# LorenzoNajt/FlipComplexityEmpirical

Measured on AMD Instinct MI355X. Metric: flip proposals/sec (node) 40x40 grid k=2, 1/2/4/8 MI355X; % LDS/HBM roofline, higher is better.
Workload: dtype int8

## Files before the change

flipcomplexityempirical_amd/csrc/fc_capi.cpp:

```cpp
#include <algorithm>
#include <cstdio>
#include <cstdlib>
#include <cstring>
#include <memory>
#include <new>
#include <string>
#include <vector>

#include "fc_run.h"

struct fc_graph {
    fc::HostGraph h;
};

namespace {

constexpr int kWaveSlots = 64;
thread_local std::string g_err;
thread_local char g_seed_kname[96] = {0};

}

int fc::fail(int code, const std::string &msg) {
    g_err = msg;
// ... 305 lines not shown
    if (!r) return fail(FC_ERR_ARG, "fc_run_set_tape: null run");
    if (r->d_sbits && tape && n_draws > 0)
        return fail(FC_ERR_ARG, "fc_run_set_tape: replay tapes need the node stream (FC_STREAM_NODE)");
    HIP_TRY(hipSetDevice(r->p.device));
    r->d_tape.release();
    r->tape_draws = 0;
    if (!tape || n_draws <= 0) return FC_OK;
    if (int rc = r->d_tape.upload(tape, (size_t)r->n_chains * (size_t)n_draws * 6)) return rc;
    r->tape_draws = n_draws;
    return FC_OK;
}

int fc_run_set_initial_wait(fc_run *r, const uint32_t *words) {
    if (!r || !words) return fail(FC_ERR_ARG, "fc_run_set_initial_wait: null argument");
    if (!(r->p.diag_mask & FC_DIAG_WAIT)) return fail(FC_ERR_ARG, "fc_run_set_initial_wait: FC_DIAG_WAIT is off");
    if (r->p.proposal == FC_PROPOSE_RECOM) return fail(FC_ERR_UNSUPPORTED, "fc_run_set_initial_wait: flip runs only");
    std::vector<fc::ChainScalars> sc;
    if (int rc = download_scalars(r, 0, r->n_chains, sc)) return rc;
    for (const auto &s : sc)
        if (s.steps != 0 || s.draw != 0) return fail(FC_ERR_ARG, "fc_run_set_initial_wait: a chain has stepped");
    for (int32_t c = 0; c < r->n_chains; ++c) {
        fc::ChainScalars &s = sc[c];
        const int64_t w = fc::geom_from(fc::u53(words[2 * c], words[2 * c + 1]), r->log1mp[s.nb]);
        s.sum_wait += w - s.wait_cur;
        s.wait_cur = w;
    }
    HIP_TRY(hipMemcpy(r->d_sc, sc.data(), sc.size() * sizeof(sc[0]), hipMemcpyHostToDevice));
    return FC_OK;
}

#ifdef FC_PHASE_PROF
static int dump_prof(fc_run *r, hipStream_t s) {
    if (const char *path = std::getenv("FC_PROF_OUT")) {
        std::vector<int64_t> h((size_t)r->n_chains * fc::kProfSlots);
        HIP_TRY(hipStreamSynchronize(s));
        HIP_TRY(hipMemcpy(h.data(), r->d_prof, h.size() * 8, hipMemcpyDeviceToHost));
        if (FILE *f = std::fopen(path, "ab")) {
            std::fwrite(h.data(), 8, h.size(), f);
            std::fclose(f);
        }
    }
    return FC_OK;
}
#endif

static fc::KParams flip_params(const fc_run *r, int64_t n_steps, int64_t max_draws) {
    fc::KParams k{};
    k.graph = r->d_graph;
    k.ring_eid = r->d_ring_eid;
    k.n = r->g.n;
    k.n_edges = r->g.n_edges;
    k.n_chains = r->n_chains;
    k.k = r->p.k;
    k.popk = r->d_popk;
    k.all_exact = r->g.n_exact == r->g.n ? 1 : 0;
    k.dgraph = r->dgraph ? 1 : 0;
    k.mcnt = r->d_mcnt;
    k.ngk = r->d_ngk;
    k.wmax = r->wmax > 0 ? r->wmax : 1;
    k.wdyn = r->p.k > 2 && r->wmax <= 0 ? 1 : 0;
    k.nfh = r->d_nfh;
    k.band = r->d_sbits ? 1 : 0;
    k.sbits = r->d_sbits;
    k.band_step0 = 1;
    while (k.band_step0 * 2 < r->words) k.band_step0 *= 2;
    k.chain_lds_bytes = r->chain_lds_bytes;
    k.words = r->words;
    k.lab_words = fc::bfs_lab_words(r->g.n);
    k.lemire_thresh = (uint32_t)((1ull << 32) % (uint64_t)r->g.n);
    k.chain_id_offset = r->p.chain_id_offset;
    k.seed_lo = (uint32_t)r->p.seed;
    k.seed_hi = (uint32_t)(r->p.seed >> 32);
    k.pop_lo = (int32_t)r->p.pop_lo;
    k.pop_hi = (int32_t)r->p.pop_hi;
    k.n_steps = n_steps;
    k.max_draws = max_draws > 0 ? max_draws : 65536 * std::max<int64_t>(n_steps, 1);
    k.assign = r->d_assign;
    k.fcnt = r->d_fcnt;
    k.sc = r->d_sc;
    k.thresh = r->d_thresh;
    k.log1mp = r->d_log1mp;
    k.labels = r->d_labels;
    k.diag = r->p.diag_mask;
    k.flags = r->p.flags;
    k.cut_hist = r->d_cut_hist;
    k.nb_hist = r->d_nb_hist;
    k.nb_w = r->nb_w;
    k.nb_pairs = (r->p.flags & FC_FLAG_NB_PAIRS) && r->p.k > 2;
    k.edge_acc = r->d_edge_acc;
    k.num_flips = r->d_num_flips;
    k.part_sum = r->d_part_sum;
    k.last_flipped = r->d_last_flipped;
    k.flip_count = r->d_flip_count;
    k.occ_acc = r->d_occ_acc;
    k.last_accept = r->d_last_accept;
    k.trace = r->d_trace;
    k.trace_chains = r->p.trace_chains;
    k.trace_cap = r->p.trace_cap;
    k.tape = r->d_tape;
    k.tape_draws = r->tape_draws;
    k.events = r->d_events;
    k.ev_cap = r->ev_cap;
    k.hit_lo = r->p.hit_lo;
    k.hit_hi = r->p.hit_hi;
    k.nsub = r->tune.nsub;
    k.hit_stop = r->tune.hit_stop;
    k.par_min = r->tune.par_min;
    k.multi_flip = r->tune.multi ? r->mf_marks : 0;
    k.wait_q = r->tune.wait_q;
    k.wpb = r->tune.wpb;
    k.coop = r->tune.coop ? 1 : 0;
    k.variant = r->variant ? 1 : 0;
    k.accept = r->p.accept;
    k.con_valid = r->p.con_valid;
    k.con_accept = r->p.con_accept;
    if (r->variant) k.par_min = kWaveSlots + 1;
    for (int i = 0; i < 3; ++i) {
        k.prio_nb[i] = r->tune.prio_div[0] > 0 && r->p.k == 2 ? k.n / r->tune.prio_div[i] : 0;
        k.prio_th[i] = r->tune.prio_th[i];
    }
    return k;
}

static fc::RecomParams recom_params(const fc_run *r, int64_t n_steps, int64_t max_draws, int64_t *prof) {
    fc::RecomParams q{};
    q.graph = r->d_graph;
    q.nbe = r->d_nbe;
    q.eslot = r->d_eslot;
    q.nb_d = r->nb_d;
    q.eu = r->d_eu;
    q.ev = r->d_ev;
    q.n = r->g.n;
    q.n_edges = r->g.n_edges;
    q.n_chains = r->n_chains;
    q.chain_lds_bytes = r->chain_lds_bytes;
    q.chain_id_offset = r->p.chain_id_offset;
    q.seed_lo = (uint32_t)r->p.seed;
    q.seed_hi = (uint32_t)(r->p.seed >> 32);
    q.pop_lo = (int32_t)r->p.pop_lo;
    q.pop_hi = (int32_t)r->p.pop_hi;
    q.pop_target = r->p.recom_pop_target;
    q.epsilon = r->p.recom_epsilon;
    q.node_repeats = r->p.recom_node_repeats > 0 ? r->p.recom_node_repeats : 1;
    q.max_attempts = r->p.recom_max_attempts > 0 ? r->p.recom_max_attempts : 10000;
    q.n_steps = n_steps;
    q.max_draws = max_draws > 0 ? max_draws : 1024 * std::max<int64_t>(n_steps, 1);
    q.assign = r->d_assign;
    q.sc = r->d_sc;
    q.accept_thresh = r->d_recom_thresh;
    q.trace = (fc_recom_record *)r->d_trace.get();
    q.trace_chains = r->p.trace_chains;
    q.trace_cap = r->p.trace_cap;
    q.prof = prof;
    return q;
}

static int take_event_slot(fc_run *r, size_t *slot) {
    if (r->n_launch_events < r->launch_events.size()) {
        *slot = (r->ev_head + r->n_launch_events) % r->launch_events.size();
        ++r->n_launch_events;
    } else if (r->launch_events.size() < fc::kMaxLaunchEvents) {
        hipEvent_t a, b;
        HIP_TRY(hipEventCreate(&a));
        HIP_TRY(hipEventCreate(&b));
        r->launch_events.emplace_back(a, b);
        *slot = r->launch_events.size() - 1;
        ++r->n_launch_events;
// ... 180 lines not shown
```

flipcomplexityempirical_amd/csrc/fc_device.h:

```cpp
#pragma once
#include <hip/hip_runtime.h>
#include <stdint.h>

#include "fc_internal.h"
#include "fc_philox.h"
#include "fc_ring.h"

namespace fc {
namespace dev {

__device__ __forceinline__ void compiler_fence() { asm volatile("" ::: "memory"); }
__device__ __forceinline__ void wave_sync() { asm volatile("s_waitcnt lgkmcnt(0)" ::: "memory"); }

#ifdef FC_PHASE_PROF
#ifdef FC_PHASE_SYNC
#define FC_STAMP(t)                                                    \
    asm volatile("s_waitcnt vmcnt(0) lgkmcnt(0)" ::: "memory");        \
    const int64_t t = (int64_t)__builtin_amdgcn_s_memtime()
#else
#define FC_STAMP(t) const int64_t t = (int64_t)__builtin_amdgcn_s_memtime()
#endif
#define FC_PROF(i, x) \
    do { if (lane == 0) atomicAdd((unsigned long long *)&prof_acc[i], (unsigned long long)(int64_t)(x)); } while (0)
#else
// ... 7 lines not shown
__device__ __forceinline__ int rl32(int x, int lane) { return __builtin_amdgcn_readlane(x, lane); }
__device__ __forceinline__ uint32_t rlu(uint32_t x, int lane) { return (uint32_t)__builtin_amdgcn_readlane((int)x, lane); }

__device__ __forceinline__ int64_t rl64(int64_t x, int lane) {
    const uint32_t lo = rlu((uint32_t)x, lane), hi = rlu((uint32_t)((uint64_t)x >> 32), lane);
    return (int64_t)(((uint64_t)hi << 32) | lo);
}
template <typename... T>
__device__ __forceinline__ void wave_sum64_all(T &...x) {
#pragma unroll
    for (int off = 32; off >= 1; off >>= 1) ((x += __shfl_xor((long long)x, off)), ...);
}
__device__ __forceinline__ int64_t wave_sum64(int64_t x) {
    wave_sum64_all(x);
    return x;
}

template <int CTRL>
__device__ __forceinline__ int32_t dpp_pair(int32_t x) {
    return __builtin_amdgcn_update_dpp(x, x, CTRL, 0xf, 0xf, false);
}
constexpr int kQuadSwap1 = 0xB1;
constexpr int kQuadSwap2 = 0x4E;
constexpr int kRowHalfMirror = 0x141;
constexpr int kRowMirror = 0x140;

__device__ __forceinline__ int32_t row0_sum(int32_t x) {
    x += dpp_pair<kQuadSwap1>(x);
    x += dpp_pair<kQuadSwap2>(x);
    x += dpp_pair<kRowHalfMirror>(x);
    x += dpp_pair<kRowMirror>(x);
    return rl32(x, 0);
}
__device__ __forceinline__ int32_t min_lanes32(int32_t x) {
    x = min(x, dpp_pair<kQuadSwap1>(x));
    x = min(x, dpp_pair<kQuadSwap2>(x));
    x = min(x, dpp_pair<kRowHalfMirror>(x));
    x = min(x, dpp_pair<kRowMirror>(x));
    return min(rl32(x, 0), rl32(x, 16));
}

__device__ __forceinline__ int count_below(uint64_t m) {
    return (int)__builtin_amdgcn_mbcnt_hi((uint32_t)(m >> 32), __builtin_amdgcn_mbcnt_lo((uint32_t)m, 0u));
}

template <int CTRL>
__device__ __forceinline__ int dpp_mov(int x) {
    return __builtin_amdgcn_update_dpp(0, x, CTRL, 0xf, 0xf, false);
}

__device__ __forceinline__ int wave_scan_incl(int x) {
    x += dpp_mov<0x111>(x);
    x += dpp_mov<0x112>(x);
    x += dpp_mov<0x114>(x);
    x += dpp_mov<0x118>(x);
    x += __builtin_amdgcn_update_dpp(0, x, 0x142, 0xa, 0xf, false);
    x += __builtin_amdgcn_update_dpp(0, x, 0x143, 0xc, 0xf, false);
    return x;
}

__device__ __forceinline__ int select_bit64(uint64_t x, int r) {
    uint32_t y = (uint32_t)x;
    int pos = 0, c = __popc(y);
    if (r >= c) { r -= c; y = (uint32_t)(x >> 32); pos = 32; }
    c = __popc(y & 0xffffu);
    if (r >= c) { r -= c; y >>= 16; pos += 16; }
    c = __popc(y & 0xffu);
    if (r >= c) { r -= c; y >>= 8; pos += 8; }
    c = __popc(y & 0xfu);
    if (r >= c) { r -= c; y >>= 4; pos += 4; }
    c = __popc(y & 0x3u);
    if (r >= c) { r -= c; y >>= 2; pos += 2; }
    return pos + (r >= (int)(y & 1u) ? 1 : 0);
}

__device__ __forceinline__ int kth_set_bit(uint64_t x, int k) {
    for (int i = 1; i < k; ++i) x &= x - 1;
    return __builtin_ctzll(x);
}

template <int RMAX>
__device__ __forceinline__ int ring_entry(const uint32_t (&ring)[RMAX / 2], int i) {
    return (int)((ring[i >> 1] >> (16 * (i & 1))) & 0xffffu);
}

using fc::one_run;
using fc::one_run_flat;

__device__ __forceinline__ int deal_chain(const KParams &p, int lane) {
    int cc = 0;
    if (lane == 0) {
        uint32_t hw, xcc;
        asm volatile("s_getreg_b32 %0, hwreg(HW_REG_HW_ID)" : "=s"(hw));
        asm volatile("s_getreg_b32 %0, hwreg(HW_REG_XCC_ID)" : "=s"(xcc));
        const uint32_t key = ((xcc & 7u) << 12) | ((hw >> 4) & 0xfffu);
        const uint32_t slot = atomicAdd(&p.deal[key], 1u);
        const uint32_t C = (uint32_t)p.n_chains;
        for (uint32_t k = 0; k < 4; ++k) {
            const uint32_t q = (slot + k) & 3u;
            const uint32_t lo = q * C / 4u, hi = (q + 1u) * C / 4u;
            const uint32_t i = atomicAdd(&p.deal[kDealKeys + q], 1u);
            if (lo + i < hi) {
                cc = (int)p.order[lo + i];
                break;
            }
        }
    }
    return __builtin_amdgcn_readfirstlane(__shfl(cc, 0));
}

constexpr int kBfsList = 512;
struct BfsScratch {
    uint32_t *lab;
    uint32_t *mm;
    uint32_t *cm;
    int32_t *lcnt;
    uint16_t *list;
    uint64_t *vis;
    uint64_t *front;
    uint64_t *nxt;
    int lab_words;
    int W;
    int64_t *prof;
};

__device__ __forceinline__ uint32_t or_reduce(uint32_t x) {
#pragma unroll
    for (int off = 32; off >= 1; off >>= 1) x |= (uint32_t)__shfl_xor((int)x, off);
    return x;
}

template <int RMAX>
__device__ __forceinline__ bool wave_bfs(const NodeRec<RMAX> *__restrict__ G, const int8_t *a, const BfsScratch &S,
                                         int lane, int vf, int A, int my_target, int64_t &levels) {
    const int W = S.W;
    uint8_t *const lab = (uint8_t *)S.lab;
    for (int i = lane; i < W; i += kWave) {
        S.vis[i] = 0;
        S.front[i] = 0;
        S.nxt[i] = 0;
    }
    if (lane < 16) {
        S.mm[lane] = 0;
        S.cm[lane] = 1u << lane;
    }
    const bool src = my_target >= 0;
    const uint64_t SM = __ballot(src);
    const int ns = __popcll(SM);
    wave_sync();
    if (ns <= 1) return true;
    if (src) {
        const uint32_t lab_me = (uint32_t)count_below(SM);
        lab[my_target] = (uint8_t)lab_me;
        atomicOr((unsigned long long *)&S.vis[my_target >> 6], 1ull << (my_target & 63));
        S.list[lab_me] = (uint16_t)my_target;
    }
    if (lane == 0) atomicOr((unsigned long long *)&S.vis[vf >> 6], 1ull << (vf & 63));
    const uint32_t all = (uint32_t)((1ull << ns) - 1ull);
    uint32_t comp = lane < 16 ? (1u << lane) : 0u;
    bool spill_in = false;
    int fcur = ns;
    wave_sync();
    for (int cur = 0;; cur ^= 1) {
        ++levels;
        uint32_t live = 0;
        bool merged = false, spill_out = false;
// ... 387 lines not shown
```

flipcomplexityempirical_amd/csrc/fc_flip2.hip:

```cpp
#include <hip/hip_runtime.h>

#include <cstdio>
#include <cstdlib>
#include <algorithm>

#include "fc_device.h"
#include "fc_internal.h"
#include "fc_philox.h"
#include "fc_tally.h"

namespace fc {

using namespace dev;

#ifndef FC_PRIO_EVERY_LOG2
#define FC_PRIO_EVERY_LOG2 4
#endif
static_assert(sizeof(KParams) % 8 == 0, "flip2_kernel's second argument sits at sizeof(KParams)");
template <bool FULL>
__device__ __forceinline__ PhiloxKeys batch_keys(PhiloxKeys keys) {
    typedef const unsigned char __attribute__((address_space(4))) *KernArg;
    if constexpr (FULL) {
        KernArg ka = (KernArg)__builtin_amdgcn_kernarg_segment_ptr();
        asm volatile("" : "+s"(ka));
        return *(const PhiloxKeys __attribute__((address_space(4))) *)(ka + sizeof(KParams));
    } else {
        asm volatile("" : "+s"(keys));
        return keys;
    }
}

template <int RMAX, int NSUB, bool FULL, bool SEARCH, bool XTRA, bool BAND>
__global__ __launch_bounds__(256, (RMAX == 8 ? 4 : 1)) void flip2_kernel(KParams p, PhiloxKeys keys) {
    static_assert(FULL || !XTRA, "XTRA is a FULL instance");
    constexpr int kRV = BAND ? NSUB : 4;
    extern __shared__ __attribute__((aligned(16))) unsigned char smem[];
    const int lane = (int)(threadIdx.x & 63u);
    const int wv = __builtin_amdgcn_readfirstlane((int)(threadIdx.x >> 6));
    const int wave = (int)blockIdx.x * (int)(blockDim.x >> 6) + wv;
    if (wave >= p.n_chains) return;
    const int c = p.order ? deal_chain(p, lane) : wave;

    const int n = p.n;
    const int npad = (n + 15) & ~15;
    unsigned char *base = smem + (size_t)wv * p.chain_lds_bytes;
    int8_t *a = (int8_t *)base;
    uint8_t *fcnt = base + npad;
    uint64_t *T = (uint64_t *)(base + 2 * npad);
    BfsScratch bs{};
    bs.vis = (uint64_t *)(T + (2 * RMAX + 2));
    bs.front = bs.vis + p.words;
    bs.nxt = bs.front + p.words;
    bs.W = p.words;
    bs.prof = nullptr;
    uint32_t *slot = (uint32_t *)(bs.nxt + p.words);
    uint8_t *smark = (uint8_t *)(slot + 5 * 64);
    uint8_t *nmark = smark + npad;
    uint8_t *const dum = nmark + npad + (lane & 15);
#define FC_ST(cond, ref, val) (*((cond) ? (uint8_t *)&(ref) : dum) = (uint8_t)(val))
    uint64_t *q_d = (uint64_t *)(nmark + npad + 16);
    uint32_t *q_nb = (uint32_t *)(q_d + kWaitQ), *q_run = q_nb + kWaitQ;
    uint32_t *q_v = q_run + kWaitQ, *q_c = q_v + kWaitQ;
    uint64_t *misc = (uint64_t *)(q_c + kWaitQ);
    uint64_t *const sb = misc + 5;
    const NodeRec<RMAX> *__restrict__ G = (const NodeRec<RMAX> *)p.graph;

    {
        const uint4 *ga = (const uint4 *)(p.assign + (size_t)c * npad);
        const uint4 *gf = (const uint4 *)(p.fcnt + (size_t)c * npad);
        for (int i = lane; i < npad / 16; i += kWave) {
            ((uint4 *)a)[i] = ga[i];
            ((uint4 *)fcnt)[i] = gf[i];
        }
        if (lane < 2 * RMAX + 1) T[lane] = p.thresh[(size_t)c * (2 * RMAX + 1) + lane];
        for (int i = lane; i < npad / 4 + 2; i += kWave) ((uint64_t *)smark)[i] = ~0ull;
        if (BAND && lane < p.words) sb[lane] = p.sbits[(size_t)c * p.words + lane];
    }
    ChainScalars *scp = p.sc + c;
    uint64_t draw = scp->draw;
    const int64_t steps_in = scp->steps;
    int64_t trace_len = FULL ? scp->trace_len : 0;
    int64_t ev_len = FULL ? scp->ev_len : 0, hit_time = FULL ? scp->hit_time : 0;
    int cut = scp->cut, nb = scp->nb;
    int pops0 = scp->pops[0], pops1 = scp->pops[1];
    const int pop_lo = scp->pop_lo, pop_hi = scp->pop_hi;
    int ng0 = scp->ngamma[0], ng1 = scp->ngamma[1];
    int64_t wait_cur = scp->wait_cur;
    int qn = 0;
    int last_flip = scp->last_flip;
    int stuck = 0;
    int rem = (int)p.n_steps;
    uint64_t draw_cap = draw + (uint64_t)p.max_draws;
    if (XTRA && p.tape && draw_cap > (uint64_t)p.tape_draws) draw_cap = (uint64_t)p.tape_draws;
    const uint32_t chain_gid = p.chain_id_offset + (uint32_t)c;
    const bool force_bfs = (p.flags & FC_FLAG_FORCE_BFS) != 0;
    const bool want_wait = (p.diag & FC_DIAG_WAIT) != 0;
    const bool trace_on = XTRA && p.trace && c < p.trace_chains;
    const bool defer = (!FULL && !BAND) || ((want_wait || FULL) && !trace_on && !(XTRA && p.tape));

    int64_t acc_cut = 0, acc_nb = 0, acc_wait = 0, acc_cut2 = 0, acc_nb2 = 0;
    int n_acc = 0, n_ic = 0, n_ip = 0;
    int64_t cnt64 = 0;
    auto cnt_fold = [&]() {
        cnt64 += lane == 0 ? n_acc : lane == 1 ? n_ic : lane == 2 ? n_ip : 0;
        n_acc = n_ic = n_ip = 0;
    };
#ifdef FC_PHASE_PROF
    int64_t *prof_acc = (int64_t *)(base + p.chain_lds_bytes - kProfSlots * 8);
    if (lane < kProfSlots) prof_acc[lane] = 0;
#endif
    wave_sync();
    uint32_t nS = 1u, thrS = 0u;
    auto band_count = [&]() {
        const int cw = lane < p.words ? (int)__popcll(sb[lane]) : 0;
        nS = (uint32_t)rl32(wave_scan_incl(cw), kWave - 1);
        thrS = (0u - nS) % nS;
// ... 398 lines not shown
        while (pos < end) {
            FC_PROF(6, 1);
            FC_STAMP(t_it0);
#ifdef FC_PHASE_PROF
            if (first_it) FC_PROF(27, t_it0 - t_c);
            first_it = false;
#endif
            asm volatile("" : "+v"(st), "+v"(inA), "+v"(tmask), "+v"(nbr), "+v"(delta), "+v"(nA), "+v"(av), "+v"(pv),
                         "+v"(v), "+v"(off_l));
            const bool hit = (st & LF_HIT) != 0, acc = (st & LF_ACC) != 0, s_lin = (st & LF_SLIN) != 0,
                       s_cyc = (st & LF_SCYC) != 0, exact = SEARCH ? (st & LF_EXACT) != 0 : true,
                       gam = (st & LF_GAM) != 0, has = (st & LF_HAS) != 0;
            const bool prop = hit & (lane >= pos) & (lane < end);
            const bool bd = SEARCH && (st & ST_BD) != 0, br = SEARCH && (st & ST_BR) != 0, nz = nA != 0;
            const bool okT = bd ? br : (nz & s_lin);
            const bool okN = bd ? br : (nz & ((exact & gam) ? s_cyc : s_lin));
            const bool known = bd | !nz | exact | s_lin;
            const bool ok = ((av ? ng0 : ng1) > 0) ? okT : okN;
            const int pa = av ? pops1 : pops0, pb = av ? pops0 : pops1;
            const bool popok = (pa - pv >= pop_lo) & (pb + pv <= pop_hi);
            bool valid = prop & known & ok & popok;
            bool acc_now = acc;
            bool inv_contig = !ok;
            if constexpr (XTRA) {
                if (p.variant) {
                    const int gm = gam ? 1 : 0;
                    const bool b_ok = ((av ? ng1 : ng0) - gm > 0) && ((av ? ng0 : ng1) + gm > 0);
                    const bool f_ok = !(st & LF_FRZ);
                    auto pass = [&](uint32_t M) {
                        return (!(M & FC_CON_CONTIG) || ok) && (!(M & FC_CON_POP) || popok) &&
                               (!(M & FC_CON_BOUNDARY) || b_ok) && (!(M & FC_CON_FIXED) || f_ok);
                    };
                    valid = prop && known && pass(p.con_valid);
                    inv_contig = (p.con_valid & FC_CON_CONTIG) && !ok;
                    bool au = acc;
                    if (p.accept == FC_ACCEPT_UNIFORM) {
                        au = true;
                    } else if (p.accept == FC_ACCEPT_ANNEAL) {
                        int dnb_l = nA == 0 ? -1 : 0;
#pragma unroll
                        for (int i = 0; i < RMAX; ++i) {
                            const int oc = fcnt[cell[i]];
                            const bool nb_i = (nbr >> i) & 1u;
                            dnb_l += nb_i ? (int)(((inA >> i) & 1u) && oc == 0) - (int)(((tmask >> i) & 1u) && oc == 1) : 0;
                        }
                        const double bw = __longlong_as_double((long long)T[delta + RMAX]);
                        const double bound = bw * ((double)(nb + dnb_l) / (double)nb);
                        au = (double)mant53(w1, w2) * 0x1p-53 < bound;
                    }
                    acc_now = pass(p.con_accept) && au;
                }
            }
            const uint64_t C0 = __ballot(valid && acc_now);
            FC_STAMP(t_it1);
            FC_PROF(8, t_it1 - t_it0);
            if (__popcll(C0) >= p.par_min) {
                FC_PROF(12, 1);
                const bool cand0 = valid && acc;
                const int dp_l = dp_of(), dg_l = dg_of();
                const int x0 = cand0 ? dp_l : 0;
                const int P = wave_scan_incl(x0) - x0;
                const int Gp = count_below(__ballot(cand0 && dg_l > 0)) - count_below(__ballot(cand0 && dg_l < 0));
                const bool ok1 = ((av ? ng0 + Gp : ng1 - Gp) > 0) ? okT : okN;
                const int q0 = pops0 + P, q1 = pops1 - P;
                const bool valid1 = prop & known & ok1 & ((av ? q1 : q0) - pv >= pop_lo) &
                                    ((av ? q0 : q1) + pv <= pop_hi);
                const bool cand1 = valid1 && acc;
                const uint64_t MM = __ballot(prop && cand1 != cand0);
                const uint64_t UU = __ballot(prop && !known);
                int sg = end;
                if (MM) sg = min(sg, __builtin_ctzll(MM) + 1);
                const int u = UU ? __builtin_ctzll(UU) : kWave;
                if (u < sg) sg = u;
                uint64_t VAL = __ballot(valid1) & lane_range(pos, sg);
                bool last_step = false;
                if (__popcll(VAL) >= rem) {
                    sg = kth_set_bit(VAL, rem) + 1;
                    VAL &= bits_below(sg);
                    last_step = true;
                }
                const uint64_t K = __ballot(cand1) & lane_range(pos, sg);
                int x = kWave;
                bool stale_seg = false;
                if (K) {
                    const bool inK = (K >> lane) & 1ull;
                    st |= inK ? LF_WROTE : 0u;
                    bool need = inK;
                    int ms = 0xff, mk[kRV];
                    uint32_t gtm = 0xffffu, ltm = 0u;
                    for (;;) {
                        FC_PROF(21, 1);
                        FC_ST(need && ms > lane, smark[v], lane);
                        const uint32_t wm = need ? (nbr & gtm) : 0u;
#pragma unroll
                        for (int i = 0; i < RMAX; ++i) FC_ST((wm >> i) & 1u, nmark[cell[i]], lane);
                        compiler_fence();
                        ms = smark[v];
                        int mn[RMAX];
#pragma unroll
                        for (int i = 0; i < RMAX; ++i) mn[i] = nmark[cell[i]];
#pragma unroll
                        for (int r = 0; r < kRV; ++r) mk[r] = nmark[rv[r] < 0 ? 0 : (rv[r] & 0xffff)];
                        gtm = 0u;
                        ltm = 0u;
#pragma unroll
                        for (int i = 0; i < RMAX; ++i) {
                            gtm |= (uint32_t)(mn[i] > lane) << i;
                            ltm |= (uint32_t)(mn[i] < lane) << i;
                        }
                        const bool again = (ms > lane) | ((nbr & gtm) != 0u);
                        need = need & again;
                        if (!__any(need)) break;
                    }
                    FC_STAMP(t_mk);
                    FC_PROF(18, t_mk - t_it1);
                    bool conf = (ms < lane) | (inK & ((nbr & ltm) != 0u));
#pragma unroll
                    for (int i = 0; i < RMAX; ++i) conf |= (int)smark[cell[i]] < lane;
                    conf &= has;
                    const uint64_t XX = __ballot(conf && lane > pos && lane < end);
                    if (XX) {
                        x = __builtin_ctzll(XX);
                        stale_seg = true;
                        FC_PROF(13, 1);
                    }
                    int t = trunc_off;
#pragma unroll
                    for (int r = 0; r < kRV; ++r) {
                        const bool tr = (rv[r] >= 0) & (mk[r] < x) & (mk[r] < (rv[r] >> 16));
                        const uint64_t TR = __ballot(tr);
                        if (TR) t = min(t, rv_off(r, __builtin_ctzll(TR)));
                    }
                    if (t < trunc_off) {
                        trunc_off = t;
                        const int e2 = __popcll(__ballot(has && off_l < t));
                        if (e2 < x) x = e2;
                        if (e2 < end) end = e2;
                        FC_PROF(14, 1);
                    }
                }
                FC_STAMP(t_cf);
                FC_PROF(19, t_cf - t_it1);
                int ce = min(sg, x);
                bool seg_out = false;
                if constexpr (BAND) {
                    const uint64_t K0 = K & bits_below(ce);
                    if (K0) {
                        bool out = false;
                        if ((K0 >> lane) & 1ull) {
#pragma unroll
                            for (int i = 0; i < RMAX; ++i) {
                                const int u = cell[i];
                                const uint32_t oc = fcnt[u];
                                const uint64_t swd = sb[u >> 6];
                                out |= ((nbr & inA) >> i & 1u) && oc == 0u && !((swd >> (u & 63)) & 1ull);
                            }
                        }
                        const uint64_t IV = __ballot(out);
                        if (IV) {
                            ce = __builtin_ctzll(IV) + 1;
                            seg_out = true;
                            if (ce < sg) last_step = false;
                        }
                    }
                }
                if (x < sg) last_step = false;
                if (prop && lane < ce) st |= valid1 ? (cand1 ? (ST_VS | ST_AC) : ST_VS) : (ok1 ? ST_IP : ST_IC);
                rem -= __popcll(VAL & bits_below(ce));
                const uint64_t AP = K & bits_below(ce);
                if (AP) {
                    FC_PROF(7, __popcll(AP));
                    const bool me = (AP >> lane) & 1ull;
                    int oldc[RMAX];
#pragma unroll
                    for (int i = 0; i < RMAX; ++i) oldc[i] = fcnt[cell[i]];
                    compiler_fence();
                    int dnb = 0;
                    const uint32_t nbm = me ? nbr : 0u;
#pragma unroll
                    for (int i = 0; i < RMAX; ++i) {
                        const int nw = oldc[i] + 2 * (int)((inA >> i) & 1u) - 1;
                        const uint32_t nb_i = (nbm >> i) & 1u;
                        FC_ST(nb_i, fcnt[cell[i]], nw);
                        dnb += (min(nw, 1) - min(oldc[i], 1)) & -(int)nb_i;
                    }
                    FC_ST(me, *(uint8_t *)&a[v], 1 - av);
                    FC_ST(me, fcnt[v], nA);
                    const int pkd = me ? ((delta + 32) | ((dnb + 32) << 16)) : 0;
                    const int S = wave_scan_incl(pkd);
                    const int cntA = count_below(AP) + 1;
                    cut_after = me ? cut + (S & 0xffff) - 32 * cntA : cut_after;
                    nb_after = me ? nb + (S >> 16) - 32 * cntA : nb_after;
                    const int L = 63 - __builtin_clzll(AP);
                    cut = rl32(cut_after, L);
                    nb = rl32(nb_after, L);
                    const int dP = rl32(P + dp_l, L), dG = rl32(Gp + dg_l, L);
                    pops0 += dP;
                    pops1 -= dP;
                    ng0 += dG;
                    ng1 -= dG;
                    last_flip = rl32(v, L);
                    compiler_fence();
                }
                if (st & LF_WROTE) {
                    smark[v] = 0xff;
#pragma unroll
                    for (int i = 0; i < RMAX; ++i) nmark[cell[i]] = 0xff;
                    st &= ~LF_WROTE;
                }
                FC_STAMP(t_sg1);
                FC_PROF(11, t_sg1 - t_it1);
                pos = ce;
                if (BAND && seg_out) rebuild = true;
                if (last_step) {
                    end = pos;
                    target_hit = true;
                    break;
                }
                if (BAND && seg_out) {
                    end = pos;
                    trunc_off = rl32(off_l, pos - 1) + 1;
                    break;
                }
                if (pos >= end) break;
                if (stale_seg && AP) {
                    reeval(pos, -1, 0u);
                    FC_STAMP(t_sg2);
                    FC_PROF(29, t_sg2 - t_sg1);
                    continue;
                }
                if (SEARCH && u == pos) {
                    const bool res = run_bfs(u);
                    if (lane == u) st |= ST_BD | (res ? ST_BR : 0u);
                }
                FC_STAMP(t_sg3);
                FC_PROF(29, t_sg3 - t_sg1);
                continue;
            }
            const uint64_t VAL = __ballot(valid);
            const uint64_t EV = C0 | __ballot(prop && !known);
            const int f = EV ? __builtin_ctzll(EV) : end;
            const uint64_t segv = VAL & bits_below(f);
            const int nvalid = __popcll(segv);
            const uint32_t bits = valid ? ST_VS : (inv_contig ? ST_IC : ST_IP);
            if (nvalid >= rem) {
                const int e = kth_set_bit(segv, rem);
                st |= (prop & (lane <= e)) ? bits : 0u;
                rem = 0;
                end = e + 1;
                target_hit = true;
                break;
            }
            st |= (prop & (lane < f)) ? bits : 0u;
            rem -= nvalid;
            pos = f;
            if (f >= end) {
                FC_STAMP(t_fx);
                FC_PROF(25, t_fx - t_it1);
                break;
            }
            if (SEARCH && !((VAL >> f) & 1ull)) {
                const bool res = run_bfs(f);
                if (lane == f) st |= ST_BD | (res ? ST_BR : 0u);
                continue;
            }
            FC_PROF(7, 1);
            FC_STAMP(t_ap0);
            FC_PROF(9, t_ap0 - t_it1);
            const int vf = rl32(v, f), Af = rl32(av, f), pvf = rl32(pv, f), df = rl32(delta, f);
            const uint32_t inAf = rlu(inA, f), nbrf = rlu(nbr, f), tmf = rlu(tmask, f);
            const bool gamf = rl32((int)gam, f) != 0;
            uint32_t rw[RMAX / 2];
#pragma unroll
            for (int k2 = 0; k2 < RMAX / 2; ++k2) rw[k2] = rlu(rec.ring[k2], f);
            uint32_t sel = rw[0];
#pragma unroll
            for (int k2 = 1; k2 < RMAX / 2; ++k2) sel = ((lane >> 1) == k2) ? rw[k2] : sel;
            const int my_e = (int)((sel >> (16 * (lane & 1))) & 0xffffu);
            const bool is_nbr = lane < RMAX && ((nbrf >> lane) & 1u);
            const int dlt = (int)((inAf >> lane) & 1u) - (int)((tmf >> lane) & 1u);
            const int old = fcnt[my_e];
            FC_ST(is_nbr, fcnt[my_e], old + dlt);
            const bool enter = is_nbr & (dlt > 0) & (old == 0);
            const bool leave = is_nbr & (dlt < 0) & (old == 1);
            bool outS = false;
            if constexpr (BAND) {
                const uint64_t swd = sb[my_e >> 6];
                outS = enter && !((swd >> (my_e & 63)) & 1ull);
            }
            if (lane == 0) {
// ... 220 lines not shown
                }
                trace_len += __popcll(PM);
            }
        }
        if (!defer && ACCM) wait_cur = rl64(my_wait, 63 - __builtin_clzll(ACCM));
        int consumed;
        if (target_hit) {
            consumed = rl32(off_l, end - 1) + 1;
        } else {
            consumed = end < ns ? rl32(off_l, end) : gen;
            if (trunc_off < consumed) consumed = trunc_off;
        }
        draw += (uint64_t)consumed;
        if constexpr (BAND) {
            if (rebuild) {
                FC_STAMP(t_rb0);
                band_rebuild();
                FC_STAMP(t_rb1);
                FC_PROF(22, 1);
                FC_PROF(23, t_rb1 - t_rb0);
            }
        }
        FC_PROF(24, ns);
        compiler_fence();
        FC_STAMP(t_e);
        FC_PROF(4, t_e - t_d);
    }
    if (defer && qn > 0) wait_flush();
    FC_STAMP(t_loop1);
    FC_PROF(0, t_loop1 - t_loop0);
    if (p.ctime && lane == 0) p.ctime[c] = (uint32_t)min(draw - scp->draw, (uint64_t)0xffffffffu);
    if (p.eta && rem == 0 && lane == 0) {
        const uint64_t el = __builtin_amdgcn_s_memrealtime() - misc[0];
        atomicMax(&p.eta[p.eta_parity], (uint32_t)min(el * 1024ull / (uint64_t)max((int)p.n_steps, 1), 0xffffffffull));
    }
#ifdef FC_PHASE_PROF
    wave_sync();
    if (p.prof && lane == 0)
        for (int i = 0; i < kProfSlots; ++i) p.prof[(size_t)c * kProfSlots + i] = prof_acc[i];
#endif

    {
        uint4 *ga = (uint4 *)(p.assign + (size_t)c * npad);
        uint4 *gf = (uint4 *)(p.fcnt + (size_t)c * npad);
        for (int i = lane; i < npad / 16; i += kWave) {
            ga[i] = ((const uint4 *)a)[i];
            gf[i] = ((const uint4 *)fcnt)[i];
        }
        if (BAND && lane < p.words) p.sbits[(size_t)c * p.words + lane] = sb[lane];
    }
    cnt_fold();
    const int taken = (int)p.n_steps - rem;
    const int64_t cnt_acc = rl64(cnt64, 0), cnt_ic = rl64(cnt64, 1), cnt_ip = rl64(cnt64, 2);
    const int64_t cnt_prop = (int64_t)taken + cnt_ic + cnt_ip;
    wave_sum64_all(acc_cut, acc_nb, acc_wait, acc_cut2, acc_nb2);
    if (FULL && p.tl_len && lane == 0) p.tl_len[c] = (int64_t)misc[3];
    if (lane == 0) {
        scp->draw = draw;
        scp->steps = steps_in + taken;
        scp->proposals += cnt_prop;
        scp->accepted += cnt_acc;
        scp->inv_contig += cnt_ic;
        scp->inv_pop += cnt_ip;
        if (FULL) {
            scp->trace_len = trace_len;
            scp->ev_len = ev_len;
            scp->hit_time = hit_time;
        }
        scp->sum_cut += acc_cut;
        scp->sum_nb += acc_nb;
        scp->sum_wait += acc_wait;
        scp->sum_cut2 += acc_cut2;
        scp->sum_nb2 += acc_nb2;
        scp->cut = cut;
        scp->nb = nb;
        scp->pops[0] = pops0;
        scp->pops[1] = pops1;
        scp->ngamma[0] = ng0;
        scp->ngamma[1] = ng1;
        scp->wait_cur = wait_cur;
        scp->last_flip = last_flip;
        scp->stuck = stuck;
    }
}

int launch_flip2(const KParams &p, const uint32_t *pkeys, int ring_max, void *stream, char *name, size_t name_cap) {
    const int wpb = p.wpb;
    const int blocks = (p.n_chains + wpb - 1) / wpb;
    const size_t lds = (size_t)p.chain_lds_bytes * wpb;
    hipStream_t s = (hipStream_t)stream;
    const dim3 grid(blocks), block(kWave * wpb);
    const PhiloxKeys keys = (PhiloxKeys)(uintptr_t)pkeys;
    const bool full = p.tape || p.trace || (p.diag & ~(uint32_t)FC_DIAG_WAIT) || p.hit_lo <= p.hit_hi || p.variant;
    const bool xtra = p.tape || p.trace || p.variant;
    const bool search = !p.all_exact || (p.flags & FC_FLAG_FORCE_BFS);
#define FC_LAUNCH2B(R, S, F, X, Y, B)                                                                      \
    do {                                                                                                    \
        if (name)                                                                                           \
            snprintf(name, name_cap, "fc::flip2_kernel<%d, %d, %s, %s, %s, %s>", R, S, F ? "true" : "false", \
                     X ? "true" : "false", Y ? "true" : "false", B ? "true" : "false");                    \
        launch_lds(flip2_kernel<R, S, F, X, Y, B>, grid, block, lds, s, p, keys);                           \
    } while (0)
#define FC_LAUNCH2(R, S, F, X, Y)                        \
    do {                                                 \
        if (p.band) FC_LAUNCH2B(R, S, F, X, Y, true);    \
        else FC_LAUNCH2B(R, S, F, X, Y, false);          \
    } while (0)
#define FC_SEARCH2(R, S, F, Y)                    \
    do {                                          \
        if (search) FC_LAUNCH2(R, S, F, true, Y);  \
        else FC_LAUNCH2(R, S, F, false, Y);        \
    } while (0)
#define FC_FULL2(R, S)                                \
    do {                                              \
        if (xtra) FC_SEARCH2(R, S, true, true);        \
        else if (full) FC_SEARCH2(R, S, true, false);  \
        else FC_SEARCH2(R, S, false, false);           \
    } while (0)
#define FC_NSUB2(R)                                \
    switch (p.nsub) {                              \
        case 1: FC_FULL2(R, 1); break;             \
        case 2: FC_FULL2(R, 2); break;             \
        case 4: FC_FULL2(R, 4); break;             \
        default: return (int)hipErrorInvalidValue; \
    }
    if (ring_max == 8) {
        FC_NSUB2(8)
    } else if (ring_max == 16) {
        FC_NSUB2(16)
    } else {
        return (int)hipErrorInvalidValue;
    }
#undef FC_NSUB2
#undef FC_FULL2
#undef FC_SEARCH2
#undef FC_LAUNCH2
#undef FC_LAUNCH2B
    return (int)hipGetLastError();
}

}
```

flipcomplexityempirical_amd/csrc/fc_graph.cpp:

```cpp
#include <algorithm>
#include <cmath>
#include <cstring>
#include <numeric>
#include <unordered_map>

#include "fc_internal.h"

namespace fc {
namespace {

struct Dart {
    int32_t from, to;
};

inline double cross(double ax, double ay, double bx, double by) { return ax * by - ay * bx; }

bool segments_intersect(const double *p1, const double *p2, const double *p3, const double *p4) {
    auto orient = [](const double *a, const double *b, const double *c) {
        double v = cross(b[0] - a[0], b[1] - a[1], c[0] - a[0], c[1] - a[1]);
        return (v > 1e-12) - (v < -1e-12);
    };
    auto on_seg = [](const double *a, const double *b, const double *c) {
        return std::min(a[0], b[0]) - 1e-12 <= c[0] && c[0] <= std::max(a[0], b[0]) + 1e-12 &&
               std::min(a[1], b[1]) - 1e-12 <= c[1] && c[1] <= std::max(a[1], b[1]) + 1e-12;
// ... 211 lines not shown
                } else {
                    ++n_breaks;
                    if (f == outer) outer_pos = (int32_t)ent.size() - 1;
                }
            }
            const int32_t L = (int32_t)ent.size();
            int32_t start = 0;
            if (n_breaks > 0) {
                int32_t bpos = outer_pos;
                if (bpos < 0) for (int32_t j = 0; j < L; ++j) if (!lnk[j]) { bpos = j; break; }
                start = (bpos + 1) % L;
            }
            if (L > 16) return "graph: link ring longer than 16 entries";
            for (int32_t j = 0; j < L; ++j) {
                const int32_t s = (start + j) % L;
                ring[v].push_back(ent[s]);
                if (isn[s]) nbr[v] |= 1u << j;
                if (lnk[s]) link[v] |= 1u << j;
            }
            const bool closed = n_breaks == 0;
            const bool gamma_open = n_breaks == 1 && outer_pos >= 0 && gamma[v] && g.outer_simple;
            exact[v] = global_ok && L >= 2 && (closed || gamma_open);
        }
    } else {
        for (int32_t v = 0; v < n; ++v) {
            const int32_t d = g.row_ptr[v + 1] - g.row_ptr[v];
            for (int32_t j = 0; j < d; ++j) {
                ring[v].push_back(g.col_idx[g.row_ptr[v] + j]);
                nbr[v] |= 1u << j;
            }
            const int32_t n_links = d >= 3 ? d : d - 1;
            for (int32_t j = 0; j < n_links; ++j)
                if (adjacent(ring[v][j], ring[v][(j + 1) % d])) link[v] |= 1u << j;
        }
    }

    for (int32_t v = 0; v < n; ++v) {
        for (size_t j = 0; j < ring[v].size(); ++j) {
            if (nbr[v] >> j & 1u) continue;
            const int32_t x = ring[v][j];
            if (std::find(ring[x].begin(), ring[x].end(), v) != ring[x].end()) continue;
            const int32_t L = (int32_t)ring[v].size();
            std::vector<int32_t> ent;
            uint32_t nn = 0, ll = 0;
            for (int32_t q = 0, o = 0; q < L; ++q) {
                if (q == (int32_t)j) continue;
                ent.push_back(ring[v][q]);
                if (nbr[v] >> q & 1u) nn |= 1u << o;
                if ((link[v] >> q & 1u) && (q + 1) % L != (int32_t)j) ll |= 1u << o;
                ++o;
            }
            ring[v] = ent;
            nbr[v] = nn;
            link[v] = ll;
            exact[v] = 0;
            --j;
        }
    }

    int32_t rmax = 0;
    for (int32_t v = 0; v < n; ++v) rmax = std::max<int32_t>(rmax, (int32_t)ring[v].size());
    g.ring_max = rmax <= 8 ? 8 : 16;
    g.ring.assign((size_t)n * g.ring_max, 0);
    g.ring_eid.assign((size_t)n * g.ring_max, -1);
    g.meta.assign(n, 0);
    std::unordered_map<int64_t, int32_t> eid;
    eid.reserve(2 * (size_t)g.n_edges);
    for (int32_t e = 0; e < g.n_edges; ++e) eid[(int64_t)g.eu[e] * n + g.ev[e]] = e;
    for (int32_t v = 0; v < n; ++v) {
        const int32_t L = (int32_t)ring[v].size();
        for (int32_t j = 0; j < g.ring_max; ++j) {
            const int32_t x = j < L ? ring[v][j] : v;
            g.ring[(size_t)v * g.ring_max + j] = x;
            if (j < L && (nbr[v] >> j & 1u)) {
                int32_t a = std::min(v, x), b = std::max(v, x);
                g.ring_eid[(size_t)v * g.ring_max + j] = eid[(int64_t)a * n + b];
            }
        }
        uint64_t m = (uint64_t)L;
        if (exact[v]) m |= kMetaExact;
        if (gamma[v] && g.outer_simple) m |= kMetaGamma;
        m |= (uint64_t)nbr[v] << kMetaNbrShift;
        m |= (uint64_t)link[v] << kMetaLinkShift;
        g.meta[v] = m;
        g.n_exact += exact[v] ? 1 : 0;
        g.n_gamma += (gamma[v] && g.outer_simple) ? 1 : 0;
    }
    return "";
}

}
```

flipcomplexityempirical_amd/csrc/fc_internal.h:

```cpp
#pragma once

#include <stddef.h>
#include <stdint.h>

#include <string>
#include <vector>

#include "../../include/flipchain.h"
#include "fc_replay.h"

namespace fc {

constexpr int kWave = 64;
constexpr int kWavesPerBlock = 4;
constexpr int kBigChainLds = 16 * 1024;
inline int bfs_lab_words(int n) { return ((n + 3) / 4 + 1) & ~1; }
inline int bfs_bytes(int n) { return 4 * bfs_lab_words(n) + 128 + 16 + 2 * 2 * 512 + 24 * ((n + 63) / 64); }
inline int waves_per_block(int chain_lds_bytes) { return chain_lds_bytes > kBigChainLds ? 1 : kWavesPerBlock; }
constexpr int kMaxK = 2;
constexpr int kMaxKGeneral = 32;
constexpr int kMaxKDistrictRule = 31;
inline int dgraph_lds_bytes(int k) { return 4 * k * k + 4 * 32 + 4 * 32; }
constexpr int hb_bytes(int ring_max) { return ring_max == 8 ? 256 : 128; }

constexpr uint64_t kMetaLenMask = 0xffull;
constexpr uint64_t kMetaExact = 1ull << 8;
constexpr uint64_t kMetaGamma = 1ull << 9;
constexpr uint64_t kMetaFrozen = 1ull << 10;
constexpr int kMetaNbrShift = 16;
constexpr int kMetaLinkShift = 32;

template <int RMAX>
struct alignas(16) NodeRec {
    uint64_t meta;
    int32_t pop;
    int32_t deg;
    uint32_t ring[RMAX / 2];
};
static_assert(sizeof(NodeRec<8>) == 32, "NodeRec<8> must be 32 B");
static_assert(sizeof(NodeRec<16>) == 48, "NodeRec<16> must be 48 B");

struct HostGraph {
    int32_t n = 0, n_edges = 0, ring_max = 8, max_degree = 0;
    std::vector<int32_t> row_ptr, col_idx, pop;
    std::vector<double> pos;
    std::vector<int32_t> eu, ev;
    std::vector<int32_t> ring;
    std::vector<uint64_t> meta;
    std::vector<int32_t> ring_eid;
    int32_t n_exact = 0, n_gamma = 0;
    bool planar = false, outer_simple = false, connected = false;
};

std::string build_host_graph(int32_t n, const int32_t *row_ptr, const int32_t *col_idx,
                             const int32_t *pop, const double *pos_xy, uint32_t flags, HostGraph &g);

struct ChainScalars {
    uint64_t draw;
    int64_t steps, proposals, accepted, inv_contig, inv_pop;
    int64_t sum_cut, sum_nb, sum_wait, sum_cut2, sum_nb2;
    int64_t wait_cur;
    int64_t bfs_calls, bfs_levels;
    int64_t trace_len;
    int64_t ev_len;
    int64_t hit_time;
    int64_t ser_t0;
    int32_t cut, nb;
    int32_t pops[kMaxK];
    int32_t ngamma[kMaxK];
    int32_t last_flip;
    int32_t stuck;
    int32_t ser_cut0, ser_nb0;
    int32_t pop_lo, pop_hi;
};

struct KParams {
    const void *graph;
    const int32_t *ring_eid;
    int32_t n, n_edges, n_chains, k;
    int32_t chain_lds_bytes;
    int32_t words;
    int32_t lab_words;
    uint32_t lemire_thresh;
    uint32_t chain_id_offset;
    uint32_t seed_lo, seed_hi;
    int32_t pop_lo, pop_hi;
    int64_t n_steps;
    int64_t max_draws;
    int8_t *assign;
    uint8_t *fcnt;
    ChainScalars *sc;
    const uint64_t *thresh;
    const double *log1mp;
    const int32_t *labels;
    uint32_t diag;
    uint32_t flags;
    int64_t *cut_hist;
    int64_t *nb_hist;
    int32_t nb_w;
    int32_t nb_pairs;
    int64_t *edge_acc;
    int64_t *num_flips;
    int64_t *part_sum;
    int64_t *last_flipped;
    int64_t *flip_count;
    int64_t *occ_acc;
    int64_t *last_accept;
    fc_record *trace;
    int32_t trace_chains;
    int64_t trace_cap;
    const uint32_t *tape;
    int64_t tape_draws;
    int32_t *popk;
// ... 123 lines not shown
```

Baseline: 21.46 billion.

## Use compact four-neighbor list for mark and count updates on degree-4 graphs

The host now precomputes, per node, the ring positions of up to four true neighbors and packs them into spare high bits of the node metadata. When every node has at most four neighbors, a flag selects a new kernel instantiation that gathers those four cell indices once per segment. It then performs neighbor-mark stores and loads and face-count updates over four entries instead of the full ring of eight. This is meant to cut LDS traffic and instructions in the conflict-resolution and accept loops on grid graphs, at the cost of extra byte-permute selects and one more kernel instantiation.

```diff
diff --git a/flipcomplexityempirical_amd/csrc/fc_capi.cpp b/flipcomplexityempirical_amd/csrc/fc_capi.cpp
--- a/flipcomplexityempirical_amd/csrc/fc_capi.cpp
+++ b/flipcomplexityempirical_amd/csrc/fc_capi.cpp
@@ -411,7 +411,12 @@
     k.log1mp = r->d_log1mp;
     k.labels = r->d_labels;
     k.diag = r->p.diag_mask;
-    k.flags = r->p.flags;
+    k.flags = r->p.flags & ~fc::kFlagNbr4;
+    {
+        bool nbr4 = true;
+        for (uint64_t m : r->g.meta) nbr4 = nbr4 && __builtin_popcount((uint32_t)(m >> fc::kMetaNbrShift) & 0xffffu) <= 4;
+        if (nbr4) k.flags |= fc::kFlagNbr4;
+    }
     k.cut_hist = r->d_cut_hist;
     k.nb_hist = r->d_nb_hist;
     k.nb_w = r->nb_w;
diff --git a/flipcomplexityempirical_amd/csrc/fc_device.h b/flipcomplexityempirical_amd/csrc/fc_device.h
--- a/flipcomplexityempirical_amd/csrc/fc_device.h
+++ b/flipcomplexityempirical_amd/csrc/fc_device.h
@@ -113,6 +113,18 @@
 template <int RMAX>
 __device__ __forceinline__ int ring_entry(const uint32_t (&ring)[RMAX / 2], int i) {
     return (int)((ring[i >> 1] >> (16 * (i & 1))) & 0xffffu);
+}
+
+template <int RMAX>
+__device__ __forceinline__ int ring_entry_at(const uint32_t (&ring)[RMAX / 2], uint32_t pos) {
+    const uint32_t sel = 0x0c0c0100u + (pos & 3u) * 0x0202u;
+    uint32_t e = __builtin_amdgcn_perm(ring[1], ring[0], sel);
+#pragma unroll
+    for (int k = 1; k < RMAX / 4; ++k) {
+        const uint32_t q = __builtin_amdgcn_perm(ring[2 * k + 1], ring[2 * k], sel);
+        e = ((pos >> 2) == (uint32_t)k) ? q : e;
+    }
+    return (int)e;
 }
 
 using fc::one_run;
diff --git a/flipcomplexityempirical_amd/csrc/fc_flip2.hip b/flipcomplexityempirical_amd/csrc/fc_flip2.hip
--- a/flipcomplexityempirical_amd/csrc/fc_flip2.hip
+++ b/flipcomplexityempirical_amd/csrc/fc_flip2.hip
@@ -3,6 +3,7 @@
 #include <cstdio>
 #include <cstdlib>
 #include <algorithm>
+#include <type_traits>
 
 #include "fc_device.h"
 #include "fc_internal.h"
@@ -30,8 +31,20 @@
     }
 }
 
-template <int RMAX, int NSUB, bool FULL, bool SEARCH, bool XTRA, bool BAND>
-__global__ __launch_bounds__(256, (RMAX == 8 ? 4 : 1)) void flip2_kernel(KParams p, PhiloxKeys keys) {
+struct NbrCells {
+    static constexpr int N = 4;
+    uint32_t w[2];
+    __device__ __forceinline__ int operator[](int i) const { return (int)((w[i >> 1] >> (16 * (i & 1))) & 0xffffu); }
+};
+template <int RMAX>
+struct RingCells {
+    static constexpr int N = RMAX;
+    const int (&c)[RMAX];
+    __device__ __forceinline__ int operator[](int i) const { return c[i]; }
+};
+
+template <int RMAX, int NSUB, bool FULL, bool SEARCH, bool XTRA, bool BAND, bool LIST>
+__device__ __forceinline__ void flip2_body(const KParams &p, PhiloxKeys keys) {
     static_assert(FULL || !XTRA, "XTRA is a FULL instance");
     constexpr int kRV = BAND ? NSUB : 4;
     extern __shared__ __attribute__((aligned(16))) unsigned char smem[];
@@ -596,8 +609,46 @@
                 const uint64_t K = __ballot(cand1) & lane_range(pos, sg);
                 int x = kWave;
                 bool stale_seg = false;
+                NbrCells nc;
+                const RingCells<RMAX> rc{cell};
+                uint32_t nm = 0u;
+                auto nbr_bits = [&]() { return LIST ? nm : nbr; };
+                auto ina_bits = [&]() { return LIST ? nm >> 16 : inA; };
+                auto marks_put = [&](const auto &cl, uint32_t wm) {
+                    constexpr int N = std::decay_t<decltype(cl)>::N;
+#pragma unroll
+                    for (int i = 0; i < N; ++i) FC_ST((wm >> i) & 1u, nmark[cl[i]], lane);
+                };
+                auto marks_get = [&](const auto &cl, uint32_t &gt, uint32_t &lt) {
+                    constexpr int N = std::decay_t<decltype(cl)>::N;
+                    int mn[N];
+#pragma unroll
+                    for (int i = 0; i < N; ++i) mn[i] = nmark[cl[i]];
+                    gt = 0u;
+                    lt = 0u;
+#pragma unroll
+                    for (int i = 0; i < N; ++i) {
+                        gt |= (uint32_t)(mn[i] > lane) << i;
+                        lt |= (uint32_t)(mn[i] < lane) << i;
+                    }
+                };
                 if (K) {
                     const bool inK = (K >> lane) & 1ull;
+                    if constexpr (LIST) {
+                        uint32_t npos = (uint32_t)(rec.meta >> kMetaPosShift);
+                        asm volatile("" : "+v"(npos));
+                        nm = (1u << min((int)__popc(nbr), 4)) - 1u;
+                        uint32_t e[4];
+#pragma unroll
+                        for (int i = 0; i < 4; ++i) {
+                            const uint32_t ps = (npos >> (4 * i)) & 15u;
+                            e[i] = (uint32_t)ring_entry_at<RMAX>(rec.ring, ps);
+                            nm |= ((inA >> ps) & 1u) << (16 + i);
+                        }
+                        nc.w[0] = e[0] | (e[1] << 16);
+                        nc.w[1] = e[2] | (e[3] << 16);
+                        asm volatile("" : "+v"(nc.w[0]), "+v"(nc.w[1]));
+                    }
                     st |= inK ? LF_WROTE : 0u;
                     bool need = inK;
                     int ms = 0xff, mk[kRV];
@@ -605,30 +656,22 @@
                     for (;;) {
                         FC_PROF(21, 1);
                         FC_ST(need && ms > lane, smark[v], lane);
-                        const uint32_t wm = need ? (nbr & gtm) : 0u;
-#pragma unroll
-                        for (int i = 0; i < RMAX; ++i) FC_ST((wm >> i) & 1u, nmark[cell[i]], lane);
+                        const uint32_t wm = need ? (nbr_bits() & gtm) : 0u;
+                        if constexpr (LIST) marks_put(nc, wm);
+                        else marks_put(rc, wm);
                         compiler_fence();
                         ms = smark[v];
-                        int mn[RMAX];
-#pragma unroll
-                        for (int i = 0; i < RMAX; ++i) mn[i] = nmark[cell[i]];
 #pragma unroll
                         for (int r = 0; r < kRV; ++r) mk[r] = nmark[rv[r] < 0 ? 0 : (rv[r] & 0xffff)];
-                        gtm = 0u;
-                        ltm = 0u;
-#pragma unroll
-                        for (int i = 0; i < RMAX; ++i) {
-                            gtm |= (uint32_t)(mn[i] > lane) << i;
-                            ltm |= (uint32_t)(mn[i] < lane) << i;
-                        }
-                        const bool again = (ms > lane) | ((nbr & gtm) != 0u);
+                        if constexpr (LIST) marks_get(nc, gtm, ltm);
+                        else marks_get(rc, gtm, ltm);
+                        const bool again = (ms > lane) | ((nbr_bits() & gtm) != 0u);
                         need = need & again;
                         if (!__any(need)) break;
                     }
                     FC_STAMP(t_mk);
                     FC_PROF(18, t_mk - t_it1);
-                    bool conf = (ms < lane) | (inK & ((nbr & ltm) != 0u));
+                    bool conf = (ms < lane) | (inK & ((nbr_bits() & ltm) != 0u));
 #pragma unroll
                     for (int i = 0; i < RMAX; ++i) conf |= (int)smark[cell[i]] < lane;
                     conf &= has;
@@ -685,19 +728,24 @@
                 if (AP) {
                     FC_PROF(7, __popcll(AP));
                     const bool me = (AP >> lane) & 1ull;
-                    int oldc[RMAX];
-#pragma unroll
-                    for (int i = 0; i < RMAX; ++i) oldc[i] = fcnt[cell[i]];
-                    compiler_fence();
                     int dnb = 0;
-                    const uint32_t nbm = me ? nbr : 0u;
-#pragma unroll
-                    for (int i = 0; i < RMAX; ++i) {
-                        const int nw = oldc[i] + 2 * (int)((inA >> i) & 1u) - 1;
-                        const uint32_t nb_i = (nbm >> i) & 1u;
-                        FC_ST(nb_i, fcnt[cell[i]], nw);
-                        dnb += (min(nw, 1) - min(oldc[i], 1)) & -(int)nb_i;
-                    }
+                    const uint32_t nbm = me ? nbr_bits() : 0u;
+                    auto counts = [&](const auto &cl) {
+                        constexpr int N = std::decay_t<decltype(cl)>::N;
+                        int oldc[N];
+#pragma unroll
+                        for (int i = 0; i < N; ++i) oldc[i] = fcnt[cl[i]];
+                        compiler_fence();
+#pragma unroll
+                        for (int i = 0; i < N; ++i) {
+                            const int nw = oldc[i] + 2 * (int)((ina_bits() >> i) & 1u) - 1;
+                            const uint32_t nb_i = (nbm >> i) & 1u;
+                            FC_ST(nb_i, fcnt[cl[i]], nw);
+                            dnb += (min(nw, 1) - min(oldc[i], 1)) & -(int)nb_i;
+                        }
+                    };
+                    if constexpr (LIST) counts(nc);
+                    else counts(rc);
                     FC_ST(me, *(uint8_t *)&a[v], 1 - av);
                     FC_ST(me, fcnt[v], nA);
                     const int pkd = me ? ((delta + 32) | ((dnb + 32) << 16)) : 0;
@@ -718,8 +766,13 @@
                 }
                 if (st & LF_WROTE) {
                     smark[v] = 0xff;
-#pragma unroll
-                    for (int i = 0; i < RMAX; ++i) nmark[cell[i]] = 0xff;
+                    if constexpr (LIST) {
+#pragma unroll
+                        for (int i = 0; i < 4; ++i) nmark[nc[i]] = 0xff;
+                    } else {
+#pragma unroll
+                        for (int i = 0; i < RMAX; ++i) nmark[cell[i]] = 0xff;
+                    }
                     st &= ~LF_WROTE;
                 }
                 FC_STAMP(t_sg1);
@@ -1106,6 +1159,17 @@
         scp->last_flip = last_flip;
         scp->stuck = stuck;
     }
+}
+
+template <int RMAX, int NSUB, bool FULL, bool SEARCH, bool XTRA, bool BAND>
+__global__ __launch_bounds__(256, (RMAX == 8 ? 4 : 1)) void flip2_kernel(KParams p, PhiloxKeys keys) {
+    if constexpr (RMAX == 8 && !FULL && !SEARCH && !BAND) {
+        if (p.flags & kFlagNbr4) {
+            flip2_body<RMAX, NSUB, FULL, SEARCH, XTRA, BAND, true>(p, keys);
+            return;
+        }
+    }
+    flip2_body<RMAX, NSUB, FULL, SEARCH, XTRA, BAND, false>(p, keys);
 }
 
 int launch_flip2(const KParams &p, const uint32_t *pkeys, int ring_max, void *stream, char *name, size_t name_cap) {
diff --git a/flipcomplexityempirical_amd/csrc/fc_graph.cpp b/flipcomplexityempirical_amd/csrc/fc_graph.cpp
--- a/flipcomplexityempirical_amd/csrc/fc_graph.cpp
+++ b/flipcomplexityempirical_amd/csrc/fc_graph.cpp
@@ -317,6 +317,7 @@
         if (gamma[v] && g.outer_simple) m |= kMetaGamma;
         m |= (uint64_t)nbr[v] << kMetaNbrShift;
         m |= (uint64_t)link[v] << kMetaLinkShift;
+        m |= meta_nbr_positions(nbr[v]);
         g.meta[v] = m;
         g.n_exact += exact[v] ? 1 : 0;
         g.n_gamma += (gamma[v] && g.outer_simple) ? 1 : 0;
diff --git a/flipcomplexityempirical_amd/csrc/fc_internal.h b/flipcomplexityempirical_amd/csrc/fc_internal.h
--- a/flipcomplexityempirical_amd/csrc/fc_internal.h
+++ b/flipcomplexityempirical_amd/csrc/fc_internal.h
@@ -29,6 +29,21 @@
 constexpr uint64_t kMetaFrozen = 1ull << 10;
 constexpr int kMetaNbrShift = 16;
 constexpr int kMetaLinkShift = 32;
+constexpr int kMetaPosShift = 48;
+constexpr uint32_t kMetaPosNone = 15u;
+constexpr uint32_t kFlagNbr4 = 1u << 31;
+inline uint64_t meta_nbr_positions(uint32_t nbr) {
+    uint64_t pos = 0;
+    for (int i = 0; i < 4; ++i) {
+        uint32_t p = kMetaPosNone;
+        if (nbr) {
+            p = (uint32_t)__builtin_ctz(nbr);
+            nbr &= nbr - 1u;
+        }
+        pos |= (uint64_t)p << (4 * i);
+    }
+    return pos << kMetaPosShift;
+}
 
 template <int RMAX>
 struct alignas(16) NodeRec {
```

Result: faster. 22.26 billion, median of 6 (+3.7%).
